# facebookresearch/mbrl-lib

Measured on AMD Instinct MI355X. Metric: candidate-steps/sec (pop×particles×horizon / plan) per CEM iter; plans/sec, higher is better.
Workload: dtype f32

## Files before the change

mbrl-lib_amd/csrc/cem.hpp:

```cpp
#pragma once
#include <type_traits>

#include "common.hpp"

namespace hipets {

struct CemDev {
    int n_env;
    int pop, H, A, D;
    int K;
    float alpha, one_minus_alpha;
    int return_mean, clipped, unbiased;
    const float* totals = nullptr;
    int P = 0;
    const int* elite_in = nullptr;
};

__device__ __forceinline__ float philox_trunc_normal(uint32_t idx_lo, uint32_t idx_hi, uint64_t seed, uint64_t stream) {
    for (uint32_t attempt = 0; attempt < 64; ++attempt) {
        const Philox4 r = philox4x32_10(idx_lo, idx_hi, attempt, (uint32_t)stream, (uint32_t)seed,
                                        (uint32_t)(seed >> 32) ^ (uint32_t)(stream >> 32) ^ 0x5EED5EEDu);
        float n0, n1, n2, n3;
        box_muller(r.x, r.y, n0, n1);
        if (fabsf(n0) <= 2.0f) return n0;
        if (fabsf(n1) <= 2.0f) return n1;
        box_muller(r.z, r.w, n2, n3);
        if (fabsf(n2) <= 2.0f) return n2;
        if (fabsf(n3) <= 2.0f) return n3;
    }
    return 0.0f;
}

__device__ __forceinline__ float philox_normal(uint32_t idx_lo, uint32_t idx_hi, uint64_t seed, uint64_t stream) {
    const Philox4 r = philox4x32_10(idx_lo, idx_hi, 0u, (uint32_t)stream, (uint32_t)seed,
                                    (uint32_t)(seed >> 32) ^ (uint32_t)(stream >> 32) ^ 0x5EED5EEDu);
    float n0, n1;
    box_muller(r.x, r.y, n0, n1);
    return n0;
}

__global__ void cem_sample_kernel(const CemDev p, const float* __restrict__ mu, const float* __restrict__ disp,
                                  const float* __restrict__ lower, const float* __restrict__ upper,
                                  const float* __restrict__ z_in, unsigned long long seed, unsigned long long stream,
                                  float* __restrict__ population) {
    const long long i = (long long)blockIdx.x * blockDim.x + threadIdx.x;
    if (i >= (long long)p.n_env * p.pop * p.D) return;
    const int d = (int)(i % p.D);
    const int env = (int)(i / ((long long)p.pop * p.D));
    const float m = mu[env * p.D + d], v = disp[env * p.D + d], lb = lower[d], ub = upper[d];
    float x;
    if (p.clipped) {
        const float z = z_in ? z_in[i] : philox_normal((uint32_t)i, (uint32_t)(i >> 32), seed, stream);
        x = m + v * z;
        x = x > lb ? x : lb;
        x = x < ub ? x : ub;
    } else {
        const float lbd = (m - lb) / 2.0f, ubd = (ub - m) / 2.0f;
        const float mv = fminf(lbd * lbd, ubd * ubd);
        const float cv = fminf(mv, v);
        const float z = z_in ? z_in[i] : philox_trunc_normal((uint32_t)i, (uint32_t)(i >> 32), seed, stream);
        x = z * sqrtf(cv) + m;
    }
    population[i] = x;
}

#ifndef HIPETS_REFIT_SKIP
#define HIPETS_REFIT_SKIP 0
#endif
constexpr int kRefitThreads = 1024;
constexpr int kMaxPop = 8192;
constexpr int kRefitScratchBytes = 12288;
constexpr int kSelectMaxK = 1024;
constexpr int kRankSortMax = 640;

__global__ __launch_bounds__(kRefitThreads) void cem_refit_kernel(const CemDev p, float* values, const float* population, float* mu,
                                                                 float* disp, float* best_value, float* best_solution,
                                                                 int* elite_idx_out) {
    extern __shared__ __attribute__((aligned(16))) char smem[];
    {
        const int env = blockIdx.y;
        values += (size_t)env * p.pop;
        if (p.totals && !(HIPETS_REFIT_SKIP & 1)) {
            const float* tot = p.totals + (size_t)env * p.pop * p.P;
            for (int i = threadIdx.x; i < p.pop; i += kRefitThreads) {
                float s = 0.f;
                for (int q0 = 0; q0 < p.P; q0 += 8) {
                    float tv[8];
#pragma unroll
                    for (int u = 0; u < 8; ++u) tv[u] = tot[(size_t)i * p.P + min(q0 + u, p.P - 1)];
#pragma unroll
                    for (int u = 0; u < 8; ++u)
                        if (q0 + u < p.P) s += tv[u];
                }
                values[i] = s / (float)p.P;
            }
        }
        population += (size_t)env * p.pop * p.D;
        mu += (size_t)env * p.D;
        disp += (size_t)env * p.D;
        best_value += env;
        best_solution += (size_t)env * p.D;
        if (elite_idx_out) elite_idx_out += (size_t)env * p.K;
    }
    const int* const elite_in = p.elite_in ? p.elite_in + (size_t)blockIdx.y * p.K : nullptr;
    int n2 = 1;
    while (n2 < p.pop) n2 <<= 1;
    float* key = reinterpret_cast<float*>(smem);
    int* idx = reinterpret_cast<int*>(smem + (size_t)n2 * 4);
    const int tid = threadIdx.x;
    for (int i = tid; i < n2; i += kRefitThreads) {
        float v = -INFINITY;
        if (i < p.pop) {
            v = values[i];
            if (v != v) { v = -1e-10f; values[i] = v; }
        }
        key[i] = v;
        idx[i] = i < p.pop ? i : 0x7FFFFFFF;
    }
    __syncthreads();
    if (elite_in) {
        auto in_range = [&](const int e) { return e < 0 ? 0 : (e >= p.pop ? p.pop - 1 : e); };
        const float top_key = key[in_range(elite_in[0])];
        __syncthreads();
        for (int k = tid; k < p.K; k += kRefitThreads) idx[k] = in_range(elite_in[k]);
        if (tid == 0) key[0] = top_key;
        __syncthreads();
    } else if (HIPETS_REFIT_SKIP & 2) {
    } else if (p.pop <= kRankSortMax) {
        for (int i = tid; i < p.pop; i += kRefitThreads) {
            const float ki = key[i];
            int rank = 0;
#pragma unroll 8
            for (int j = 0; j < i; ++j) rank += key[j] >= ki;
#pragma unroll 8
            for (int j = i + 1; j < p.pop; ++j) rank += key[j] > ki;
            idx[i] = rank;
        }
        __syncthreads();
        int* pos = reinterpret_cast<int*>(smem + (size_t)n2 * 8);
        for (int i = tid; i < p.pop; i += kRefitThreads) pos[idx[i]] = i;
        __syncthreads();
        float top_key = key[pos[0]];
        __syncthreads();
        for (int i = tid; i < p.pop; i += kRefitThreads) idx[i] = pos[i];
        if (tid == 0) key[0] = top_key;
        __syncthreads();
    } else if (p.K <= kSelectMaxK) {
// ... 70 lines not shown
        }
        __syncthreads();
        if (my_pos >= 0) idx[my_pos] = my_id;
        if (my_pos == 0) key[0] = my_key;
        __syncthreads();
    } else
    for (int k = 2; k <= n2; k <<= 1) {
        for (int j = k >> 1; j > 0; j >>= 1) {
            for (int i = tid; i < n2; i += kRefitThreads) {
                const int ixj = i ^ j;
                if (ixj > i) {
                    const float ka = key[i], kb = key[ixj];
                    const int ia = idx[i], ib = idx[ixj];
                    const bool a_first = (ka > kb) || (ka == kb && ia < ib);
                    const bool up = (i & k) == 0;
                    if (up ? !a_first : a_first) {
                        key[i] = kb; key[ixj] = ka;
                        idx[i] = ib; idx[ixj] = ia;
                    }
                }
            }
            __syncthreads();
        }
    }
    if (elite_idx_out && blockIdx.x == 0)
        for (int k = tid; k < p.K; k += kRefitThreads) elite_idx_out[k] = idx[k];

    const float top = key[0];
    const bool improved = blockIdx.x == 0 && top > best_value[0];
    const int top_i = idx[0];
    __syncthreads();

    double* red = reinterpret_cast<double*>(smem + (size_t)n2 * 8);
    const int nb = (int)gridDim.x, bx = (int)blockIdx.x;
    const int Dslice = (((p.D + nb - 1) / nb + 63) / 64) * 64;
    const int d_lo = bx * Dslice, d_hi = min(p.D, d_lo + Dslice);
    int parts = kRefitThreads / Dslice;
    parts = parts < 1 ? 1 : (parts > 8 ? 8 : parts);
    const int G = kRefitThreads / parts;
    const int part = tid / G, dloc = tid % G;
    const int nu = (p.K + parts - 1) / parts;
    auto sweep = [&](const int base, auto nu_tag, auto hold_tag) __attribute__((always_inline)) {
        constexpr int NU = decltype(nu_tag)::value;
        constexpr bool HOLD = decltype(hold_tag)::value;
        const int d = base + dloc;
        const bool live = d < d_hi && part < parts;
        float mu_old = 0.f, disp_old = 0.f;
        float xv[NU];
        double s = 0.0;
        if (live) {
            if (part == 0) { mu_old = mu[d]; disp_old = disp[d]; }
            for (int k0 = part; k0 < (HOLD ? part + 1 : p.K); k0 += parts * NU) {
#pragma unroll
                for (int u = 0; u < NU; ++u) xv[u] = population[(size_t)idx[min(k0 + u * parts, p.K - 1)] * p.D + d];
#pragma unroll
                for (int u = 0; u < NU; ++u)
                    if (k0 + u * parts < p.K) s += (double)xv[u];
            }
        }
        red[tid] = s;
        __syncthreads();
        double mean = 0.0;
        if (live) {
            for (int q = 0; q < parts; ++q) mean += red[q * G + dloc];
            mean /= (double)p.K;
        }
        __syncthreads();
        double ss = 0.0;
        if (live) {
            for (int k0 = part; k0 < (HOLD ? part + 1 : p.K); k0 += parts * NU) {
                if constexpr (!HOLD) {
#pragma unroll
                    for (int u = 0; u < NU; ++u) xv[u] = population[(size_t)idx[min(k0 + u * parts, p.K - 1)] * p.D + d];
                }
#pragma unroll
                for (int u = 0; u < NU; ++u)
                    if (k0 + u * parts < p.K) {
                        const double dv = (double)xv[u] - mean;
                        ss += dv * dv;
                    }
            }
        }
        red[tid] = ss;
        __syncthreads();
// ... 4 lines not shown
            const float new_mu = (float)mean;
            const float new_disp = p.clipped ? (float)sqrt(var) : (float)var;
            mu[d] = p.alpha * mu_old + p.one_minus_alpha * new_mu;
            disp[d] = p.alpha * disp_old + p.one_minus_alpha * new_disp;
        }
        __syncthreads();
    };
    constexpr int kBestHold = 4;
    float best_row[kBestHold];
    const bool best_held = p.D <= kBestHold * kRefitThreads;
    if (improved && best_held) {
#pragma unroll
        for (int u = 0; u < kBestHold; ++u) best_row[u] = population[(size_t)top_i * p.D + min(tid + u * kRefitThreads, p.D - 1)];
    }
    for (int base = d_lo; base < ((HIPETS_REFIT_SKIP & 4) ? d_lo : d_hi); base += G) {
        using T = std::true_type;
        using F = std::false_type;
        if (nu <= 2) sweep(base, std::integral_constant<int, 2>{}, T{});
        else if (nu <= 4) sweep(base, std::integral_constant<int, 4>{}, T{});
        else if (nu <= 8) sweep(base, std::integral_constant<int, 8>{}, T{});
        else if (nu <= 16) sweep(base, std::integral_constant<int, 16>{}, T{});
        else sweep(base, std::integral_constant<int, 16>{}, F{});
    }
    if (improved) {
        if (best_held) {
#pragma unroll
            for (int u = 0; u < kBestHold; ++u)
                if (tid + u * kRefitThreads < p.D) best_solution[tid + u * kRefitThreads] = best_row[u];
        } else {
            for (int d = tid; d < p.D; d += kRefitThreads) best_solution[d] = population[(size_t)top_i * p.D + d];
        }
        if (tid == 0) best_value[0] = top;
    }
}

inline int refit_blocks(const int D) { return D <= 128 ? 1 : (D + 127) / 128 > 8 ? 8 : (D + 127) / 128; }

__global__ void cem_init_kernel(const CemDev p, const float* x0, const float* lower, const float* upper, float* mu,
                                float* disp, float* best_value) {
    const int i = blockIdx.x * blockDim.x + threadIdx.x;
    if (i < p.n_env * p.D) {
        const int d = i % p.D;
        mu[i] = x0[i];
        const float w = upper[d] - lower[d];
        disp[i] = p.clipped ? 1.0f : (w * w) / 16.0f;
    }
    if (i < p.n_env) best_value[i] = -INFINITY;
}

}
```

mbrl-lib_amd/csrc/hipets.hip:

```cpp
#include <hip/hip_runtime.h>
#include <hip/hip_ext.h>

#include <dlfcn.h>

#include <algorithm>
#include <cmath>
#include <cstdarg>
#include <cstdio>
#include <cstring>
#include <string>
#include <vector>

#include "../../include/hipets.h"
#include "cem.hpp"
#include "launch.hpp"
#include "optim.hpp"
#include "residency.hpp"
#include "rollout_helpers.hpp"
#include "rollout_smem.hpp"
#include "train.hpp"

using namespace hipets;

namespace {
// ... 48 lines not shown
        cap = 0;
    }
    template <typename T>
    T* as() const { return reinterpret_cast<T*>(p); }
};

}

struct hipets_engine {
    int device = 0;
    int num_cu = 256;
    size_t lds_max = 160 * 1024;
    bool has_model = false;
    ModelDev md{};
    int ensemble_size = 0;
    DevBuf w3pack;
    DevBuf wpack, bpack, layer_meta, norm_mean, norm_std, min_lv, max_lv, no_delta, members;
    DevBuf s0, state, totals, term;
    DevBuf exchange, step_keys, plan_keys;
    struct HostStage { void* p = nullptr; size_t cap = 0; hipEvent_t done = nullptr; bool used = false; };
    HostStage stage[4];
    int stage_next = 0;
    uint32_t tag_base = 0;
    uint64_t plan_keys_seed = 0, plan_keys_first = 0;
    int plan_keys_count = 0, plan_keys_H = 0;
    int* error_flag = nullptr;
    bool persistent_ok = true;
    long long poll_ticks = 20000000ll;
    DevBuf census;
    hipStream_t last_stream = nullptr;
    bool last_stream_set = false;
    hipEvent_t last_done = nullptr;
    DevBuf mu, disp, population, values, best_value, best_solution, past_action, kept, elite_idx, keep_idx;
    void* comm = nullptr;
    int comm_rank = 0, comm_world = 1;
    DevBuf shard_values, gathered;
    bool has_planet = false;
    bool planet_static = false;
    PlanetDev pd{};
    DevBuf planet_w, planet_b, planet_member, planet_ops;
    int plan_mode = HIPETS_MODE_FAST;
    bool has_trace = false;
    hipets_plan_trace trace{};
    bool timing = false;
    int timing_stride = 1;
    unsigned long long launch_counter = 0;
    std::vector<std::pair<hipEvent_t, hipEvent_t>> events;
    std::vector<std::pair<hipEvent_t, hipEvent_t>> event_pool;
    DevBuf train_slab, train_partial;
};

namespace {

KernelRec* rollout_instance(const hipets_engine* e, int R, const RolloutArgs& ra) {
    static constexpr decltype(&rollout_instance_r1) resolvers[kMaxR] = {rollout_instance_r1, rollout_instance_r2, rollout_instance_r3, rollout_instance_r4};
    if (R < 1 || R > kMaxR) return fail("unsupported rows_per_group %d (1..%d)", R, kMaxR), nullptr;
    hipError_t why = hipSuccess;
    KernelRec* k = resolvers[R - 1](e->md, ra, &why);
    const bool b3 = e->md.precision == HIPETS_PREC_BF16X3;
    if (!k && why == hipErrorNotSupported && (b3 || e->md.precision == HIPETS_PREC_BF16))
        fail("precision %s: no shape-specialised kernel instance for this model / call (SiLU, f64 normaliser, no obs preprocessing, in-kernel "
             "sampling, one of the %s layer shapes, R = %d); use precision f32", b3 ? "bf16x3" : "bf16", b3 ? "BASELINE" : "two bf16", R);
    else if (!k) fail_kind(HIPETS_ERR_RUNTIME, "rollout kernel launch failed: %s", hipGetErrorString(why));
    return k;
}

// ... 168 lines not shown
        if (sl.p) (void)hipHostFree(sl.p);
        sl.p = nullptr;
        sl.cap = 0;
        HCHECK(hipHostMalloc(&sl.p, bytes < 4096 ? 4096 : bytes, hipHostMallocDefault));
        sl.cap = bytes < 4096 ? 4096 : bytes;
    }
    if (!sl.done) HCHECK(hipEventCreateWithFlags(&sl.done, hipEventDisableTiming));
    std::memcpy(sl.p, src, bytes);
    HCHECK(hipMemcpyAsync(dst, sl.p, bytes, hipMemcpyHostToDevice, st));
    HCHECK(hipEventRecord(sl.done, st));
    sl.used = true;
    return 0;
}

int enter_stream(hipets_engine* e, hipStream_t st) {
    if (!e->last_done) HCHECK(hipEventCreateWithFlags(&e->last_done, hipEventDisableTiming));
    if (e->last_stream_set && e->last_stream != st) HCHECK(hipStreamWaitEvent(st, e->last_done, 0));
    e->last_stream = st;
    e->last_stream_set = true;
    return 0;
}
struct StreamScope {
    hipets_engine* e;
    hipStream_t st;
    ~StreamScope() {
        static const bool off = std::getenv("HIPETS_NO_STREAM_SCOPE") != nullptr;
        if (e && e->last_done && !off) (void)hipEventRecord(e->last_done, st);
    }
};
#define ENTER_STREAM(e, st)                \
    if (enter_stream((e), (st))) return 1; \
    StreamScope stream_scope_ { (e), (st) }

int plan_prologue(hipets_engine* e, const float* s0, int n_env, int H, int iters, uint64_t seed, uint64_t first_stream, hipStream_t st) {
    const ModelDev& md = e->md;
    if (e->s0.ensure((size_t)n_env * md.obs_dim * 4)) return 1;
    if (stage_h2d(e, e->s0.p, s0, (size_t)n_env * md.obs_dim * 4, st)) return 1;
    if (md.propagation == HIPETS_PROP_RANDOM_MODEL && iters >= 1 && e->plan_mode == HIPETS_MODE_DEVICE && e->persistent_ok) {
        if (e->plan_keys.ensure((size_t)iters * H * sizeof(PermKeys))) return 1;
        hipLaunchKernelGGL(step_keys_kernel, dim3((H + 63) / 64, iters), dim3(64), 0, st, e->plan_keys.as<PermKeys>(), H, (unsigned long long)seed,
                           (unsigned long long)first_stream);
        HCHECK(hipGetLastError());
        e->plan_keys_seed = seed; e->plan_keys_first = first_stream; e->plan_keys_count = iters; e->plan_keys_H = H;
    }
    return 0;
}

struct RcclId { char internal[HIPETS_COMM_ID_BYTES]; };
struct Rccl {
    void* lib = nullptr;
    int (*GetUniqueId)(void*) = nullptr;
    int (*CommInitRank)(void**, int, RcclId , int) = nullptr;
    int (*CommDestroy)(void*) = nullptr;
    int (*AllGather)(const void*, void*, size_t, int, void*, hipStream_t) = nullptr;
    const char* (*GetErrorString)(int) = nullptr;
    int (*CommCount)(void*, int*) = nullptr;
    int (*CommUserRank)(void*, int*) = nullptr;
};
Rccl g_rccl;

int rccl_load() {
    if (g_rccl.lib) return 0;
    void* lib = nullptr;
    const char* forced = std::getenv("HIPETS_RCCL_LIB");
    if (forced && forced[0]) {
        lib = dlopen(forced, RTLD_NOW | RTLD_LOCAL);
        if (!lib) return fail_kind(HIPETS_ERR_RUNTIME, "cannot load the RCCL library named by HIPETS_RCCL_LIB (%s): %s", forced, dlerror());
    }
    for (const char* name : {"librccl.so.1", "librccl.so", "/opt/rocm/lib/librccl.so"}) {
        if (lib) break;
        lib = dlopen(name, RTLD_NOW | RTLD_GLOBAL);
    }
    if (!lib) return fail_kind(HIPETS_ERR_RUNTIME, "cannot load librccl: %s", dlerror());
    g_rccl.GetUniqueId = reinterpret_cast<int (*)(void*)>(dlsym(lib, "ncclGetUniqueId"));
    g_rccl.CommInitRank = reinterpret_cast<int (*)(void**, int, RcclId, int)>(dlsym(lib, "ncclCommInitRank"));
    g_rccl.CommDestroy = reinterpret_cast<int (*)(void*)>(dlsym(lib, "ncclCommDestroy"));
// ... 80 lines not shown

int hipets_create(int device, hipets_engine** out) {
    if (!out) return fail("null out pointer");
    *out = nullptr;
    int n = 0;
    hipError_t err = hipGetDeviceCount(&n);
    if (err != hipSuccess || n <= 0)
        return fail("no HIP device visible (%s) -- libhipets has no CPU fallback", hipGetErrorString(err));
    if (device < 0 || device >= n) return fail("device %d out of range (%d visible)", device, n);
    HCHECK(hipSetDevice(device));
    hipDeviceProp_t prop;
    HCHECK(hipGetDeviceProperties(&prop, device));
    if (std::string(prop.gcnArchName).rfind("gfx950", 0) != 0)
        return fail("device %d is %s; libhipets is built for gfx950 (MI355X) only", device, prop.gcnArchName);
    auto* e = new hipets_engine();
    e->device = device;
    e->num_cu = prop.multiProcessorCount > 0 ? prop.multiProcessorCount : 256;
    e->lds_max = prop.sharedMemPerBlockOptin > 0 ? (size_t)prop.sharedMemPerBlockOptin : (size_t)prop.sharedMemPerBlock;
    if (e->lds_max > 160 * 1024) e->lds_max = 160 * 1024;
    if (hipHostMalloc(reinterpret_cast<void**>(&e->error_flag), sizeof(int), hipHostMallocMapped) != hipSuccess) e->error_flag = nullptr;
    if (e->error_flag) *e->error_flag = 0;
    const char* np = std::getenv("HIPETS_NO_PERSISTENT");
    e->persistent_ok = e->error_flag != nullptr && !(np && np[0] == '1');
    if (e->census.ensure(2 * sizeof(int))) e->persistent_ok = false;
    *out = e;
    return 0;
}

void hipets_destroy(hipets_engine* e) {
    if (!e) return;
    (void)hipSetDevice(e->device);
    if (e->comm && g_rccl.CommDestroy) (void)g_rccl.CommDestroy(e->comm);
    for (DevBuf* b : {&e->w3pack, &e->wpack, &e->bpack, &e->layer_meta, &e->norm_mean, &e->norm_std, &e->min_lv, &e->max_lv, &e->no_delta, &e->members,
                      &e->s0, &e->state, &e->totals, &e->term, &e->exchange, &e->step_keys, &e->plan_keys, &e->mu, &e->disp, &e->population, &e->values,
                      &e->best_value, &e->best_solution, &e->past_action, &e->kept, &e->elite_idx, &e->keep_idx, &e->planet_w, &e->planet_b, &e->planet_member, &e->planet_ops, &e->shard_values, &e->gathered, &e->census, &e->train_slab, &e->train_partial})
        b->release();
    for (auto& ev : e->events) { (void)hipEventDestroy(ev.first); (void)hipEventDestroy(ev.second); }
    for (auto& ev : e->event_pool) { (void)hipEventDestroy(ev.first); (void)hipEventDestroy(ev.second); }
    if (e->error_flag) (void)hipHostFree(e->error_flag);
    if (e->last_done) (void)hipEventDestroy(e->last_done);
    for (auto& sl : e->stage) {
        if (sl.p) (void)hipHostFree(sl.p);
        if (sl.done) (void)hipEventDestroy(sl.done);
    }
    delete e;
}

int hipets_set_model(hipets_engine* e, const hipets_model_desc* d, void* stream) {
    if (!e || !d) return fail("null argument");
    hipStream_t st = reinterpret_cast<hipStream_t>(stream);
    HCHECK(hipSetDevice(e->device));
    ENTER_STREAM(e, st);
    if (d->n_layers < 2 || d->n_layers > HIPETS_MAX_LAYERS) return fail("n_layers %d outside [2, %d]", d->n_layers, HIPETS_MAX_LAYERS);
    if (d->n_members < 1 || d->n_members > d->ensemble_size) return fail("n_members %d invalid for ensemble_size %d", d->n_members, d->ensemble_size);
    if (d->obs_dim < 1 || d->act_dim < 1 || d->in_dim < d->act_dim + 1 || d->hid < 1) return fail("bad dimensions");
    if (d->out_dim != d->obs_dim + (d->learned_rewards ? 1 : 0)) return fail("out_dim %d != obs_dim %d + learned_rewards %d", d->out_dim, d->obs_dim, d->learned_rewards);
    const int obs_in = d->in_dim - d->act_dim;
    const int expect_in = d->obs_process == HIPETS_OBS_CARTPOLE_PETS ? d->obs_dim + 1 : d->obs_dim;
    if (obs_in != expect_in) return fail("in_dim %d inconsistent with obs_dim %d / obs_process %d / act_dim %d", d->in_dim, d->obs_dim, d->obs_process, d->act_dim);
    if (d->reward_fn == HIPETS_REW_LEARNED && !d->learned_rewards) return fail("reward_fn LEARNED needs learned_rewards");
    if (d->reward_fn == HIPETS_REW_HALFCHEETAH && d->obs_dim < 3) return fail("halfcheetah reward needs obs_dim >= 3");
    if (d->reward_fn == HIPETS_REW_PUSHER && d->obs_dim < 20) return fail("pusher reward needs obs_dim >= 20");
    if ((d->reward_fn == HIPETS_REW_CARTPOLE || d->termination_fn == HIPETS_TERM_CARTPOLE) && d->obs_dim < 3) return fail("cartpole fns need obs_dim >= 3");
    if ((d->obs_process == HIPETS_OBS_HALFCHEETAH) && d->obs_dim < 3) return fail("halfcheetah obs_process needs obs_dim >= 3");
    if (d->obs_dim < 2 && (d->termination_fn != HIPETS_TERM_NONE || d->reward_fn == HIPETS_REW_CARTPOLE_PETS)) return fail("termination/reward fn needs obs_dim >= 2");
    if (!d->deterministic && (!d->min_logvar || !d->max_logvar)) return fail("logvar bounds missing");
    if (d->ensemble_kind != HIPETS_ENSEMBLE_GAUSSIAN_MLP && d->ensemble_kind != HIPETS_ENSEMBLE_BASIC)
// ... 458 lines not shown
        return 0;
    }
};
PlanObjective ensemble_objective(const float* s0, PlanObjective::Kind kind = PlanObjective::ENSEMBLE) {
    PlanObjective o;
    o.kind = kind;
    o.s0 = s0;
    return o;
}
PlanObjective planet_objective(const float* latent0, const float* belief0) {
    PlanObjective o;
    o.kind = PlanObjective::PLANET;
    o.latent0 = latent0;
    o.belief0 = belief0;
    return o;
}

int check_plan(const hipets_engine* e, const PlanObjective& obj, bool args, int A, int n_env, int P) {
    const bool planet = obj.is_planet();
    if (planet && !(e && e->has_planet)) return fail("engine has no PlaNet model (call hipets_planet_set_model)");
    if (!planet && !(e && e->has_model)) return fail("engine has no model (call hipets_set_model)");
    if (!args || (planet ? !(obj.latent0 && obj.belief0) : !obj.s0)) return fail("null argument");
    if (planet && A != e->pd.action) return fail("act_dim %d != model action_size %d", A, e->pd.action);
    if (!planet && A != e->md.act_dim) return fail("act_dim %d != model act_dim %d", A, e->md.act_dim);
    if (n_env < 1 || n_env > 4096) return fail("n_env %d outside [1, 4096]", n_env);
    if (planet && P < 1) return fail("bad pop/horizon/particles");
    return 0;
}

int launch_cem_refit(const CemDev& c, float* values, const float* population, float* mu, float* disp, float* best_value, float* best_solution,
                     int* elite_idx, hipStream_t st) {
    int n2 = 1;
    while (n2 < c.pop) n2 <<= 1;
    hipLaunchKernelGGL(cem_refit_kernel, dim3(refit_blocks(c.D), c.n_env), dim3(kRefitThreads), (size_t)n2 * 8 + kRefitScratchBytes, st, c, values,
                       population, mu, disp, best_value, best_solution, elite_idx);
    HCHECK(hipGetLastError());
    return 0;
}

int plan_cem_impl(hipets_engine* e, const hipets_cem_params* p, int32_t n_env, const float* x0, const float* lower, const float* upper,
                  const PlanObjective& obj, int32_t P, uint64_t seed, uint64_t plan_id, float* out, void* stream);
int plan_mppi_impl(hipets_engine* e, int32_t pop, int32_t H, int32_t A, int32_t num_iterations, double gamma, double beta, int32_t n_env,
                   float* mean, const float* lower, const float* upper, const PlanObjective& obj, int32_t P, uint64_t seed, uint64_t plan_id,
                   void* stream);
int plan_icem_impl(hipets_engine* e, const hipets_icem_params* p, int32_t n_env, const float* x0, const float* lower, const float* upper,
                   float* elite, int32_t has_elite, const int32_t* keep_idx, const PlanObjective& obj, int32_t P, uint64_t seed, uint64_t plan_id,
                   float* out, void* stream);

}

extern "C" {

int hipets_step(hipets_engine* e, const float* obs, const float* actions, int32_t B, const hipets_rollout_opts* o, float* next_obs,
                float* rewards, uint8_t* dones, void* stream) {
    if (!e || !e->has_model) return fail("engine has no model (call hipets_set_model)");
    if (!obs || !actions || !o || !next_obs || !rewards || !dones) return fail("null argument");
    if (B < 1) return fail("bad batch");
    hipStream_t st = reinterpret_cast<hipStream_t>(stream);
    HCHECK(hipSetDevice(e->device));
    ENTER_STREAM(e, st);
    const ModelDev& md = e->md;
    if (o->rows_per_group < 0 || o->rows_per_group > kMaxR) return fail("rows_per_group outside [0, %d]", kMaxR);
    if (check_member_maps(e, o, B, true)) return 1;
    if (o->mode != HIPETS_MODE_EXACT && o->mode != HIPETS_MODE_DEVICE && o->mode != HIPETS_MODE_FAST) return fail("unknown rollout mode %d", o->mode);
    RolloutArgs ra{};
    ra.pop = B; ra.P = 1; ra.H = 1; ra.B = B;
    ra.actions = actions;
// ... 203 lines not shown
    if (!e || !kept || !mu || !var || !out) return fail("null argument");
    if (keep < 1 || H < 1 || A < 1) return fail("bad keep/horizon/act_dim");
    HCHECK(hipSetDevice(e->device));
    const int n = keep * H * A;
    hipLaunchKernelGGL(icem_shift_kernel, dim3((n + 255) / 256), dim3(256), 0, reinterpret_cast<hipStream_t>(stream), 1, keep, keep, H, A, kept,
                       mu, var, end_noise, (unsigned long long)seed, (unsigned long long)stream_id, out);
    HCHECK(hipGetLastError());
    return 0;
}

int hipets_plan_cem(hipets_engine* e, const hipets_cem_params* p, const float* x0, const float* lower, const float* upper,
                    const float* s0, int32_t P, uint64_t seed, uint64_t plan_id, float* out, void* stream) {
    return hipets_plan_cem_batched(e, p, 1, x0, lower, upper, s0, P, seed, plan_id, out, stream);
}

int hipets_plan_cem_batched(hipets_engine* e, const hipets_cem_params* p, int32_t n_env, const float* x0, const float* lower,
                            const float* upper, const float* s0, int32_t P, uint64_t seed, uint64_t plan_id, float* out,
                            void* stream) {
    return plan_cem_impl(e, p, n_env, x0, lower, upper, ensemble_objective(s0), P, seed, plan_id, out, stream);
}

}

namespace {
int plan_cem_impl(hipets_engine* e, const hipets_cem_params* p, int32_t n_env, const float* x0, const float* lower, const float* upper,
                  const PlanObjective& obj, int32_t P, uint64_t seed, uint64_t plan_id, float* out, void* stream) {
    if (check_cem(p) || check_plan(e, obj, x0 && lower && upper && out, p->act_dim, n_env, P)) return 1;
    if (obj.is_sharded() && check_shards(e, p->population_size, P)) return 1;
    hipStream_t st = reinterpret_cast<hipStream_t>(stream);
    HCHECK(hipSetDevice(e->device));
    ENTER_STREAM(e, st);
    const CemDev c = make_cem(p, n_env);
    const size_t nd = (size_t)n_env * c.D, npop = (size_t)n_env * c.pop;
    if (e->mu.ensure(nd * 4) || e->disp.ensure(nd * 4) || e->best_solution.ensure(nd * 4) || e->best_value.ensure((size_t)n_env * 4 + 16) ||
        e->population.ensure(npop * c.D * 4) || e->values.ensure(npop * 4) || obj.reserve_shards(e, c.pop))
        return 1;
    LocalErr le;
    hipets_rollout_opts ro{};
    ro.mode = e->plan_mode;
    ro.seed = obj.rollout_seed(e, seed);
    ro.n_env = n_env;
    auto prologue = [&]() -> int {
        if (obj.clear_padding(e, c.pop, st)) return 1;
        hipLaunchKernelGGL(cem_init_kernel, dim3((unsigned)((nd + 255) / 256)), dim3(256), 0, st, c, x0, lower, upper, e->mu.as<float>(),
                           e->disp.as<float>(), e->best_value.as<float>());
        HCHECK(hipGetLastError());
        HCHECK(hipMemsetAsync(e->best_solution.p, 0, nd * 4, st));
        return obj.is_planet() ? 0 : plan_prologue(e, obj.s0, n_env, c.H, p->num_iterations, ro.seed, plan_id * (uint64_t)p->num_iterations, st);
    };
    le.note(prologue());
    if (!obj.is_sharded() && !le.ok()) return le.report();
    for (int i = 0; i < p->num_iterations; ++i) {
        const uint64_t sid = plan_id * (uint64_t)p->num_iterations + (uint64_t)i;
        auto sample = [&]() -> int {
            const long long n = (long long)npop * c.D;
            hipLaunchKernelGGL(cem_sample_kernel, dim3((unsigned)((n + 255) / 256)), dim3(256), 0, st, c, e->mu.as<float>(), e->disp.as<float>(),
                               lower, upper, (const float*)nullptr, (unsigned long long)seed, (unsigned long long)sid, e->population.as<float>());
            HCHECK(hipGetLastError());
            return 0;
        };
        auto refit = [&]() -> int {
            int* eidx = (e->has_trace && e->trace.elite_idx) ? e->trace.elite_idx + (size_t)i * n_env * c.K : nullptr;
            CemDev cr = c;
            obj.refit_from_totals(e, &cr, P);
            if (launch_cem_refit(cr, e->values.as<float>(), e->population.as<float>(), e->mu.as<float>(), e->disp.as<float>(), e->best_value.as<float>(),
                                 e->best_solution.as<float>(), eidx, st))
                return 1;
            return trace_iter(e, i, (int)npop, (size_t)c.D, e->population.as<float>(), e->values.as<float>(), e->mu.as<float>(), e->disp.as<float>(), st, n_env);
        };
        if (le.ok()) le.note(sample());
        ro.stream_id = sid;
        if (obj.evaluate(e, e->population.as<float>(), (int32_t)npop, c.H, P, &ro, nullptr, stream, le)) return 1;
        if (le.ok()) le.note(refit());
        if (!obj.is_sharded() && !le.ok()) break;
    }
    if (!le.ok()) return le.report();
    HCHECK(hipMemcpyAsync(out, p->return_mean_elites ? e->mu.p : e->best_solution.p, nd * 4, hipMemcpyDeviceToDevice, st));
    return 0;
}
}

extern "C" {

int hipets_plan_mppi(hipets_engine* e, int32_t pop, int32_t H, int32_t A, int32_t num_iterations, double gamma, double beta,
                     float* mean, const float* lower, const float* upper, const float* s0, int32_t P, uint64_t seed,
                     uint64_t plan_id, void* stream) {
    return hipets_plan_mppi_batched(e, pop, H, A, num_iterations, gamma, beta, 1, mean, lower, upper, s0, P, seed, plan_id, stream);
}

int hipets_plan_mppi_batched(hipets_engine* e, int32_t pop, int32_t H, int32_t A, int32_t num_iterations, double gamma, double beta,
                             int32_t n_env, float* mean, const float* lower, const float* upper, const float* s0, int32_t P,
                             uint64_t seed, uint64_t plan_id, void* stream) {
    return plan_mppi_impl(e, pop, H, A, num_iterations, gamma, beta, n_env, mean, lower, upper, ensemble_objective(s0), P, seed, plan_id, stream);
}

int hipets_plan_mppi_sharded(hipets_engine* e, int32_t pop, int32_t H, int32_t A, int32_t num_iterations, double gamma, double beta,
                             float* mean, const float* lower, const float* upper, const float* s0, int32_t P, uint64_t seed,
                             uint64_t plan_id, void* stream) {
    if (e && !e->comm) return fail("no communicator (call hipets_comm_init)");
    return plan_mppi_impl(e, pop, H, A, num_iterations, gamma, beta, 1, mean, lower, upper, ensemble_objective(s0, PlanObjective::SHARDED), P, seed, plan_id, stream);
}

}

namespace {
int plan_mppi_impl(hipets_engine* e, int32_t pop, int32_t H, int32_t A, int32_t num_iterations, double gamma, double beta, int32_t n_env,
                   float* mean, const float* lower, const float* upper, const PlanObjective& obj, int32_t P, uint64_t seed, uint64_t plan_id,
                   void* stream) {
    if (check_plan(e, obj, mean && lower && upper, A, n_env, P)) return 1;
    if (pop < 1 || pop > 12000) return fail("population_size %d outside [1, 12000]", pop);
// ... 579 lines not shown
```

Baseline: 290.4 million.

## Fuse CEM sampling into refit and pre-draw normals in a plan-begin kernel

Adds a single plan-begin kernel that initializes mu/disp/best values, samples the first population, pre-generates normals for every later iteration and builds the permutation keys. This replaces the init kernel, the memset and the separate step_keys launch. The refit kernel now also emits the next iteration's population from the pre-drawn normals, using ping-pong mu/disp/population buffers, so the per-iteration sample kernel launch goes away. The per-candidate averaging over particle totals moves into the key-load loop. The aim is fewer kernel launches and less inter-kernel gap time between rollouts, at the cost of extra memory for (iters-1) normal buffers and more refit blocks.

```diff
diff --git a/mbrl-lib_amd/csrc/cem.hpp b/mbrl-lib_amd/csrc/cem.hpp
--- a/mbrl-lib_amd/csrc/cem.hpp
+++ b/mbrl-lib_amd/csrc/cem.hpp
@@ -14,6 +14,13 @@
     const float* totals = nullptr;
     int P = 0;
     const int* elite_in = nullptr;
+    const float* z_next = nullptr;
+    float* population_next = nullptr;
+    const float* lower = nullptr;
+    const float* upper = nullptr;
+    int emit_groups = 1;
+    const float* mu_in = nullptr;
+    const float* disp_in = nullptr;
 };
 
 __device__ __forceinline__ float philox_trunc_normal(uint32_t idx_lo, uint32_t idx_hi, uint64_t seed, uint64_t stream) {
@@ -39,6 +46,27 @@
     return n0;
 }
 
+__device__ __forceinline__ float cem_draw(const int clipped, const long long i, const uint64_t seed, const uint64_t stream) {
+    return clipped ? philox_normal((uint32_t)i, (uint32_t)(i >> 32), seed, stream) : philox_trunc_normal((uint32_t)i, (uint32_t)(i >> 32), seed, stream);
+}
+
+__device__ __forceinline__ float cem_place(const int clipped, const float z, const float m, const float v, const float lb, const float ub) {
+    if (clipped) {
+        float x = m + v * z;
+        x = x > lb ? x : lb;
+        return x < ub ? x : ub;
+    }
+    const float lbd = (m - lb) / 2.0f, ubd = (ub - m) / 2.0f;
+    const float mv = fminf(lbd * lbd, ubd * ubd);
+    const float cv = fminf(mv, v);
+    return z * sqrtf(cv) + m;
+}
+
+__device__ __forceinline__ float cem_dispersion0(const int clipped, const float lb, const float ub) {
+    const float w = ub - lb;
+    return clipped ? 1.0f : (w * w) / 16.0f;
+}
+
 __global__ void cem_sample_kernel(const CemDev p, const float* __restrict__ mu, const float* __restrict__ disp,
                                   const float* __restrict__ lower, const float* __restrict__ upper,
                                   const float* __restrict__ z_in, unsigned long long seed, unsigned long long stream,
@@ -47,21 +75,35 @@
     if (i >= (long long)p.n_env * p.pop * p.D) return;
     const int d = (int)(i % p.D);
     const int env = (int)(i / ((long long)p.pop * p.D));
-    const float m = mu[env * p.D + d], v = disp[env * p.D + d], lb = lower[d], ub = upper[d];
-    float x;
-    if (p.clipped) {
-        const float z = z_in ? z_in[i] : philox_normal((uint32_t)i, (uint32_t)(i >> 32), seed, stream);
-        x = m + v * z;
-        x = x > lb ? x : lb;
-        x = x < ub ? x : ub;
-    } else {
-        const float lbd = (m - lb) / 2.0f, ubd = (ub - m) / 2.0f;
-        const float mv = fminf(lbd * lbd, ubd * ubd);
-        const float cv = fminf(mv, v);
-        const float z = z_in ? z_in[i] : philox_trunc_normal((uint32_t)i, (uint32_t)(i >> 32), seed, stream);
-        x = z * sqrtf(cv) + m;
-    }
-    population[i] = x;
+    const float z = z_in ? z_in[i] : cem_draw(p.clipped, i, seed, stream);
+    population[i] = cem_place(p.clipped, z, mu[env * p.D + d], disp[env * p.D + d], lower[d], upper[d]);
+}
+
+__global__ void cem_plan_begin_kernel(const CemDev p, const int iters, const float* __restrict__ x0, const float* __restrict__ lower,
+                                      const float* __restrict__ upper, unsigned long long seed, unsigned long long first_stream,
+                                      float* __restrict__ mu, float* __restrict__ disp, float* __restrict__ best_value,
+                                      float* __restrict__ best_solution, float* __restrict__ population, float* __restrict__ z,
+                                      PermKeys* __restrict__ keys, int keys_H, unsigned long long keys_seed) {
+    const long long n = (long long)p.n_env * p.pop * p.D;
+    const long long i = (long long)blockIdx.x * blockDim.x + threadIdx.x;
+    const int it = blockIdx.y;
+    if (keys && i < keys_H && it < iters) keys[(size_t)it * keys_H + i] = perm_round_keys(perm_key(keys_seed, first_stream + it, (unsigned)i));
+    if (i >= n) return;
+    if (it > 0) {
+        z[(size_t)(it - 1) * n + i] = cem_draw(p.clipped, i, seed, first_stream + it);
+        return;
+    }
+    const int d = (int)(i % p.D);
+    const int env = (int)(i / ((long long)p.pop * p.D));
+    const float m = x0[env * p.D + d], lb = lower[d], ub = upper[d];
+    const float v = cem_dispersion0(p.clipped, lb, ub);
+    if (iters > 0) population[i] = cem_place(p.clipped, cem_draw(p.clipped, i, seed, first_stream), m, v, lb, ub);
+    if (i < (long long)p.n_env * p.D) {
+        mu[i] = x0[i];
+        disp[i] = v;
+        best_solution[i] = 0.0f;
+    }
+    if (i < p.n_env) best_value[i] = -INFINITY;
 }
 
 #ifndef HIPETS_REFIT_SKIP
@@ -80,21 +122,6 @@
     {
         const int env = blockIdx.y;
         values += (size_t)env * p.pop;
-        if (p.totals && !(HIPETS_REFIT_SKIP & 1)) {
-            const float* tot = p.totals + (size_t)env * p.pop * p.P;
-            for (int i = threadIdx.x; i < p.pop; i += kRefitThreads) {
-                float s = 0.f;
-                for (int q0 = 0; q0 < p.P; q0 += 8) {
-                    float tv[8];
-#pragma unroll
-                    for (int u = 0; u < 8; ++u) tv[u] = tot[(size_t)i * p.P + min(q0 + u, p.P - 1)];
-#pragma unroll
-                    for (int u = 0; u < 8; ++u)
-                        if (q0 + u < p.P) s += tv[u];
-                }
-                values[i] = s / (float)p.P;
-            }
-        }
         population += (size_t)env * p.pop * p.D;
         mu += (size_t)env * p.D;
         disp += (size_t)env * p.D;
@@ -108,11 +135,28 @@
     float* key = reinterpret_cast<float*>(smem);
     int* idx = reinterpret_cast<int*>(smem + (size_t)n2 * 4);
     const int tid = threadIdx.x;
+    const bool from_totals = p.totals && !(HIPETS_REFIT_SKIP & 1);
+    const float* const tot = from_totals ? p.totals + (size_t)blockIdx.y * p.pop * p.P : nullptr;
     for (int i = tid; i < n2; i += kRefitThreads) {
         float v = -INFINITY;
         if (i < p.pop) {
-            v = values[i];
-            if (v != v) { v = -1e-10f; values[i] = v; }
+            bool store = from_totals;
+            if (from_totals) {
+                float s = 0.f;
+                for (int q0 = 0; q0 < p.P; q0 += 8) {
+                    float tv[8];
+#pragma unroll
+                    for (int u = 0; u < 8; ++u) tv[u] = tot[(size_t)i * p.P + min(q0 + u, p.P - 1)];
+#pragma unroll
+                    for (int u = 0; u < 8; ++u)
+                        if (q0 + u < p.P) s += tv[u];
+                }
+                v = s / (float)p.P;
+            } else {
+                v = values[i];
+            }
+            if (v != v) { v = -1e-10f; store = true; }
+            if (store && blockIdx.x == 0) values[i] = v;
         }
         key[i] = v;
         idx[i] = i < p.pop ? i : 0x7FFFFFFF;
@@ -249,7 +293,9 @@
     __syncthreads();
 
     double* red = reinterpret_cast<double*>(smem + (size_t)n2 * 8);
-    const int nb = (int)gridDim.x, bx = (int)blockIdx.x;
+    const int nb = (int)gridDim.x / p.emit_groups, bx = (int)blockIdx.x % nb, emit_group = (int)blockIdx.x / nb;
+    const float* const mu_in = p.mu_in ? p.mu_in + (size_t)blockIdx.y * p.D : mu;
+    const float* const disp_in = p.disp_in ? p.disp_in + (size_t)blockIdx.y * p.D : disp;
     const int Dslice = (((p.D + nb - 1) / nb + 63) / 64) * 64;
     const int d_lo = bx * Dslice, d_hi = min(p.D, d_lo + Dslice);
     int parts = kRefitThreads / Dslice;
@@ -266,7 +312,7 @@
         float xv[NU];
         double s = 0.0;
         if (live) {
-            if (part == 0) { mu_old = mu[d]; disp_old = disp[d]; }
+            if (part == 0) { mu_old = mu_in[d]; disp_old = disp_in[d]; }
             for (int k0 = part; k0 < (HOLD ? part + 1 : p.K); k0 += parts * NU) {
 #pragma unroll
                 for (int u = 0; u < NU; ++u) xv[u] = population[(size_t)idx[min(k0 + u * parts, p.K - 1)] * p.D + d];
@@ -337,9 +383,30 @@
         }
         if (tid == 0) best_value[0] = top;
     }
-}
-
-inline int refit_blocks(const int D) { return D <= 128 ? 1 : (D + 127) / 128 > 8 ? 8 : (D + 127) / 128; }
+    if (p.z_next && !(HIPETS_REFIT_SKIP & 4)) {
+        const float* __restrict__ zn = p.z_next + (size_t)blockIdx.y * p.pop * p.D;
+        float* __restrict__ pn = p.population_next + (size_t)blockIdx.y * p.pop * p.D;
+        constexpr int kWaves = kRefitThreads / 64, kFlight = 8;
+        const int first = emit_group * kWaves + (tid >> 6), stride = kWaves * p.emit_groups;
+        for (int d = d_lo + (tid & 63); d < d_hi; d += 64) {
+            const float m = mu[d], v = disp[d], lb = p.lower[d], ub = p.upper[d];
+            for (int c0 = first; c0 < p.pop; c0 += stride * kFlight) {
+                float zv[kFlight];
+#pragma unroll
+                for (int u = 0; u < kFlight; ++u) zv[u] = zn[(size_t)min(c0 + u * stride, p.pop - 1) * p.D + d];
+#pragma unroll
+                for (int u = 0; u < kFlight; ++u)
+                    if (c0 + u * stride < p.pop) pn[(size_t)(c0 + u * stride) * p.D + d] = cem_place(p.clipped, zv[u], m, v, lb, ub);
+            }
+        }
+    }
+}
+
+inline int refit_blocks(const int D) {
+    const int w = D <= 512 ? 64 : 128;
+    return (D + w - 1) / w > 8 ? 8 : (D + w - 1) / w;
+}
+inline int refit_emit_groups(const int pop) { return (pop + 63) / 64 > 8 ? 8 : (pop + 63) / 64; }
 
 __global__ void cem_init_kernel(const CemDev p, const float* x0, const float* lower, const float* upper, float* mu,
                                 float* disp, float* best_value) {
@@ -347,8 +414,7 @@
     if (i < p.n_env * p.D) {
         const int d = i % p.D;
         mu[i] = x0[i];
-        const float w = upper[d] - lower[d];
-        disp[i] = p.clipped ? 1.0f : (w * w) / 16.0f;
+        disp[i] = cem_dispersion0(p.clipped, lower[d], upper[d]);
     }
     if (i < p.n_env) best_value[i] = -INFINITY;
 }
diff --git a/mbrl-lib_amd/csrc/hipets.hip b/mbrl-lib_amd/csrc/hipets.hip
--- a/mbrl-lib_amd/csrc/hipets.hip
+++ b/mbrl-lib_amd/csrc/hipets.hip
@@ -104,6 +104,7 @@
     bool last_stream_set = false;
     hipEvent_t last_done = nullptr;
     DevBuf mu, disp, population, values, best_value, best_solution, past_action, kept, elite_idx, keep_idx;
+    DevBuf population_next, cem_normals;
     void* comm = nullptr;
     int comm_rank = 0, comm_world = 1;
     DevBuf shard_values, gathered;
@@ -338,16 +339,24 @@
     if (enter_stream((e), (st))) return 1; \
     StreamScope stream_scope_ { (e), (st) }
 
+int plan_stage_s0(hipets_engine* e, const float* s0, int n_env, hipStream_t st) {
+    if (e->s0.ensure((size_t)n_env * e->md.obs_dim * 4)) return 1;
+    return stage_h2d(e, e->s0.p, s0, (size_t)n_env * e->md.obs_dim * 4, st);
+}
+int plan_keys_reserve(hipets_engine* e, int H, int iters, uint64_t seed, uint64_t first_stream, PermKeys** keys) {
+    *keys = nullptr;
+    if (!(e->md.propagation == HIPETS_PROP_RANDOM_MODEL && iters >= 1 && e->plan_mode == HIPETS_MODE_DEVICE && e->persistent_ok)) return 0;
+    if (e->plan_keys.ensure((size_t)iters * H * sizeof(PermKeys))) return 1;
+    e->plan_keys_seed = seed; e->plan_keys_first = first_stream; e->plan_keys_count = iters; e->plan_keys_H = H;
+    *keys = e->plan_keys.as<PermKeys>();
+    return 0;
+}
 int plan_prologue(hipets_engine* e, const float* s0, int n_env, int H, int iters, uint64_t seed, uint64_t first_stream, hipStream_t st) {
-    const ModelDev& md = e->md;
-    if (e->s0.ensure((size_t)n_env * md.obs_dim * 4)) return 1;
-    if (stage_h2d(e, e->s0.p, s0, (size_t)n_env * md.obs_dim * 4, st)) return 1;
-    if (md.propagation == HIPETS_PROP_RANDOM_MODEL && iters >= 1 && e->plan_mode == HIPETS_MODE_DEVICE && e->persistent_ok) {
-        if (e->plan_keys.ensure((size_t)iters * H * sizeof(PermKeys))) return 1;
-        hipLaunchKernelGGL(step_keys_kernel, dim3((H + 63) / 64, iters), dim3(64), 0, st, e->plan_keys.as<PermKeys>(), H, (unsigned long long)seed,
-                           (unsigned long long)first_stream);
+    PermKeys* keys;
+    if (plan_stage_s0(e, s0, n_env, st) || plan_keys_reserve(e, H, iters, seed, first_stream, &keys)) return 1;
+    if (keys) {
+        hipLaunchKernelGGL(step_keys_kernel, dim3((H + 63) / 64, iters), dim3(64), 0, st, keys, H, (unsigned long long)seed, (unsigned long long)first_stream);
         HCHECK(hipGetLastError());
-        e->plan_keys_seed = seed; e->plan_keys_first = first_stream; e->plan_keys_count = iters; e->plan_keys_H = H;
     }
     return 0;
 }
@@ -494,7 +503,7 @@
     (void)hipSetDevice(e->device);
     if (e->comm && g_rccl.CommDestroy) (void)g_rccl.CommDestroy(e->comm);
     for (DevBuf* b : {&e->w3pack, &e->wpack, &e->bpack, &e->layer_meta, &e->norm_mean, &e->norm_std, &e->min_lv, &e->max_lv, &e->no_delta, &e->members,
-                      &e->s0, &e->state, &e->totals, &e->term, &e->exchange, &e->step_keys, &e->plan_keys, &e->mu, &e->disp, &e->population, &e->values,
+                      &e->s0, &e->state, &e->totals, &e->term, &e->exchange, &e->step_keys, &e->plan_keys, &e->mu, &e->disp, &e->population, &e->population_next, &e->cem_normals, &e->values,
                       &e->best_value, &e->best_solution, &e->past_action, &e->kept, &e->elite_idx, &e->keep_idx, &e->planet_w, &e->planet_b, &e->planet_member, &e->planet_ops, &e->shard_values, &e->gathered, &e->census, &e->train_slab, &e->train_partial})
         b->release();
     for (auto& ev : e->events) { (void)hipEventDestroy(ev.first); (void)hipEventDestroy(ev.second); }
@@ -1019,7 +1028,7 @@
                      int* elite_idx, hipStream_t st) {
     int n2 = 1;
     while (n2 < c.pop) n2 <<= 1;
-    hipLaunchKernelGGL(cem_refit_kernel, dim3(refit_blocks(c.D), c.n_env), dim3(kRefitThreads), (size_t)n2 * 8 + kRefitScratchBytes, st, c, values,
+    hipLaunchKernelGGL(cem_refit_kernel, dim3(refit_blocks(c.D) * c.emit_groups, c.n_env), dim3(kRefitThreads), (size_t)n2 * 8 + kRefitScratchBytes, st, c, values,
                        population, mu, disp, best_value, best_solution, elite_idx);
     HCHECK(hipGetLastError());
     return 0;
@@ -1289,50 +1298,62 @@
     ENTER_STREAM(e, st);
     const CemDev c = make_cem(p, n_env);
     const size_t nd = (size_t)n_env * c.D, npop = (size_t)n_env * c.pop;
-    if (e->mu.ensure(nd * 4) || e->disp.ensure(nd * 4) || e->best_solution.ensure(nd * 4) || e->best_value.ensure((size_t)n_env * 4 + 16) ||
-        e->population.ensure(npop * c.D * 4) || e->values.ensure(npop * 4) || obj.reserve_shards(e, c.pop))
+    const int iters = p->num_iterations;
+    const size_t nz = npop * c.D;
+    if (e->mu.ensure(2 * nd * 4) || e->disp.ensure(2 * nd * 4) || e->best_solution.ensure(nd * 4) || e->best_value.ensure((size_t)n_env * 4 + 16) ||
+        e->population.ensure(nz * 4) || e->population_next.ensure(iters > 1 ? nz * 4 : 0) ||
+        e->cem_normals.ensure(iters > 1 ? (size_t)(iters - 1) * nz * 4 : 0) || e->values.ensure(npop * 4) || obj.reserve_shards(e, c.pop))
         return 1;
     LocalErr le;
     hipets_rollout_opts ro{};
     ro.mode = e->plan_mode;
     ro.seed = obj.rollout_seed(e, seed);
     ro.n_env = n_env;
+    const uint64_t first_stream = plan_id * (uint64_t)iters;
     auto prologue = [&]() -> int {
         if (obj.clear_padding(e, c.pop, st)) return 1;
-        hipLaunchKernelGGL(cem_init_kernel, dim3((unsigned)((nd + 255) / 256)), dim3(256), 0, st, c, x0, lower, upper, e->mu.as<float>(),
-                           e->disp.as<float>(), e->best_value.as<float>());
+        PermKeys* keys = nullptr;
+        if (!obj.is_planet() && (plan_stage_s0(e, obj.s0, n_env, st) || plan_keys_reserve(e, c.H, iters, ro.seed, first_stream, &keys))) return 1;
+        hipLaunchKernelGGL(cem_plan_begin_kernel, dim3((unsigned)((nz + 255) / 256), (unsigned)std::max(iters, 1)), dim3(256), 0, st, c, iters, x0, lower,
+                           upper, (unsigned long long)seed, (unsigned long long)first_stream, e->mu.as<float>(), e->disp.as<float>(),
+                           e->best_value.as<float>(), e->best_solution.as<float>(), e->population.as<float>(), e->cem_normals.as<float>(), keys, c.H,
+                           (unsigned long long)ro.seed);
         HCHECK(hipGetLastError());
-        HCHECK(hipMemsetAsync(e->best_solution.p, 0, nd * 4, st));
-        return obj.is_planet() ? 0 : plan_prologue(e, obj.s0, n_env, c.H, p->num_iterations, ro.seed, plan_id * (uint64_t)p->num_iterations, st);
+        return 0;
     };
     le.note(prologue());
     if (!obj.is_sharded() && !le.ok()) return le.report();
-    for (int i = 0; i < p->num_iterations; ++i) {
-        const uint64_t sid = plan_id * (uint64_t)p->num_iterations + (uint64_t)i;
-        auto sample = [&]() -> int {
-            const long long n = (long long)npop * c.D;
-            hipLaunchKernelGGL(cem_sample_kernel, dim3((unsigned)((n + 255) / 256)), dim3(256), 0, st, c, e->mu.as<float>(), e->disp.as<float>(),
-                               lower, upper, (const float*)nullptr, (unsigned long long)seed, (unsigned long long)sid, e->population.as<float>());
-            HCHECK(hipGetLastError());
-            return 0;
-        };
+    float* pop_cur = e->population.as<float>();
+    float* pop_next = e->population_next.as<float>();
+    float *mu_cur = e->mu.as<float>(), *mu_new = mu_cur + nd, *disp_cur = e->disp.as<float>(), *disp_new = disp_cur + nd;
+    for (int i = 0; i < iters; ++i) {
         auto refit = [&]() -> int {
             int* eidx = (e->has_trace && e->trace.elite_idx) ? e->trace.elite_idx + (size_t)i * n_env * c.K : nullptr;
             CemDev cr = c;
             obj.refit_from_totals(e, &cr, P);
-            if (launch_cem_refit(cr, e->values.as<float>(), e->population.as<float>(), e->mu.as<float>(), e->disp.as<float>(), e->best_value.as<float>(),
-                                 e->best_solution.as<float>(), eidx, st))
+            cr.mu_in = mu_cur;
+            cr.disp_in = disp_cur;
+            if (i + 1 < iters) {
+                cr.z_next = e->cem_normals.as<float>() + (size_t)i * nz;
+                cr.population_next = pop_next;
+                cr.lower = lower;
+                cr.upper = upper;
+                cr.emit_groups = refit_emit_groups(c.pop);
+            }
+            if (launch_cem_refit(cr, e->values.as<float>(), pop_cur, mu_new, disp_new, e->best_value.as<float>(), e->best_solution.as<float>(), eidx, st))
                 return 1;
-            return trace_iter(e, i, (int)npop, (size_t)c.D, e->population.as<float>(), e->values.as<float>(), e->mu.as<float>(), e->disp.as<float>(), st, n_env);
+            return trace_iter(e, i, (int)npop, (size_t)c.D, pop_cur, e->values.as<float>(), mu_new, disp_new, st, n_env);
         };
-        if (le.ok()) le.note(sample());
-        ro.stream_id = sid;
-        if (obj.evaluate(e, e->population.as<float>(), (int32_t)npop, c.H, P, &ro, nullptr, stream, le)) return 1;
+        ro.stream_id = first_stream + (uint64_t)i;
+        if (obj.evaluate(e, pop_cur, (int32_t)npop, c.H, P, &ro, nullptr, stream, le)) return 1;
         if (le.ok()) le.note(refit());
         if (!obj.is_sharded() && !le.ok()) break;
+        std::swap(pop_cur, pop_next);
+        std::swap(mu_cur, mu_new);
+        std::swap(disp_cur, disp_new);
     }
     if (!le.ok()) return le.report();
-    HCHECK(hipMemcpyAsync(out, p->return_mean_elites ? e->mu.p : e->best_solution.p, nd * 4, hipMemcpyDeviceToDevice, st));
+    HCHECK(hipMemcpyAsync(out, p->return_mean_elites ? (void*)mu_cur : e->best_solution.p, nd * 4, hipMemcpyDeviceToDevice, st));
     return 0;
 }
 }
diff --git a/profiles/plan_seams.py b/profiles/plan_seams.py
--- /dev/null
+++ b/profiles/plan_seams.py
@@ -0,0 +1,61 @@
+#!/usr/bin/env python
+import argparse
+import collections
+import csv
+import glob
+import json
+import os
+import re
+
+
+def short(name):
+    m = re.search(r"(\w+_kernel)", name)
+    return m.group(1) if m else name.split("(")[0][:60]
+
+
+def load(dirname):
+    paths = sorted(glob.glob(os.path.join(dirname, "**", "*kernel_trace.csv"), recursive=True))
+    if not paths:
+        raise SystemExit(f"no *kernel_trace.csv under {dirname}")
+    rows = []
+    for path in paths:
+        with open(path, newline="") as f:
+            for r in csv.DictReader(f):
+                rows.append((int(r["Start_Timestamp"]), int(r["End_Timestamp"]), short(r["Kernel_Name"])))
+    rows.sort()
+    return rows
+
+
+def main():
+    ap = argparse.ArgumentParser()
+    ap.add_argument("dir")
+    ap.add_argument("--iters", type=int, default=5, help="rollouts per plan (bench.py: 5)")
+    args = ap.parse_args()
+    rows = load(args.dir)
+    per = collections.defaultdict(list)
+    for a, b, n in rows:
+        per[n].append(b - a)
+    kernels = {n: {"calls": len(v), "avg_us": round(sum(v) / len(v) / 1e3, 3), "total_us": round(sum(v) / 1e3, 1)} for n, v in sorted(per.items())}
+    is_roll = [n.startswith("rollout") for _, _, n in rows]
+    idx = [i for i, r in enumerate(is_roll) if r]
+    between = collections.Counter()
+    gaps = collections.defaultdict(list)
+    for i, j in zip(idx, idx[1:]):
+        seq = tuple(rows[k][2] for k in range(i + 1, j))
+        between[" > ".join(seq) or "(nothing)"] += 1
+        gaps[" > ".join(seq) or "(nothing)"].append(rows[j][0] - rows[i][1])
+    n_roll = len(idx)
+    plans = n_roll / args.iters if args.iters else 0
+    other_us = sum(sum(v) for n, v in per.items() if not n.startswith("rollout")) / 1e3
+    out = {
+        "kernels": kernels,
+        "rollout_dispatches": n_roll,
+        "plans": plans,
+        "non_rollout_kernel_us_per_plan": round(other_us / plans, 2) if plans else None,
+        "between_two_rollouts": {k: {"count": c, "median_gap_us": round(sorted(gaps[k])[len(gaps[k]) // 2] / 1e3, 2)} for k, c in between.most_common(8)},
+    }
+    print(json.dumps(out, indent=1))
+
+
+if __name__ == "__main__":
+    main()
```

New measurement: 291.0 million (median of 6 runs). About the same (+0.2%).
